# jondo2010/rust-ida

Hardware: AMD Instinct MI355X
Metric: Newton iters/sec (fp64), batched dense DAE N=512 B=4096 (higher is better)
Workload: dtype f64

## Files before the change

### rust-ida_amd/csrc/exp_switches.hpp

```cpp
#pragma once

#if !defined(IDAHIP_TIMING_BUILD) &&                                                                                   \
    (defined(IDAHIP_EXP_NOPRO) || defined(IDAHIP_EXP_NOUPD) || defined(IDAHIP_EXP_NOGATHER) || defined(IDAHIP_EXP_NODIAG) || \
     defined(IDAHIP_EXP_NOSWEEP) || defined(IDAHIP_STAMPS) || defined(IDAHIP_TRAIL_PIPE) || defined(IDAHIP_TRAIL_QUAD) ||   \
     defined(IDAHIP_WP_RING) || defined(IDAHIP_US_PAD) || defined(IDAHIP_SYS_UNR) || defined(IDAHIP_TRAIL_AHEAD) ||         \
     defined(IDAHIP_NT_SYS) || defined(IDAHIP_NT_SOLVE) || defined(IDAHIP_NT_FINALIZE) || defined(IDAHIP_NT_TRAIL))
#error "IDAHIP_EXP_* / IDAHIP_STAMPS / IDAHIP_TRAIL_* (IDAHIP_TRAIL_AHEAD: 0..3) / IDAHIP_WP_RING / IDAHIP_US_PAD / IDAHIP_SYS_UNR / IDAHIP_NT_* are timing-build switches: add -DIDAHIP_TIMING_BUILD (the library then reports itself as one and is not a product)"
#endif

namespace idahip {
namespace tb {

#ifdef IDAHIP_TIMING_BUILD
constexpr bool TIMING_BUILD = true;
#else
constexpr bool TIMING_BUILD = false;
#endif

#ifdef IDAHIP_EXP_NOPRO
constexpr bool NOPRO = true;
#else
constexpr bool NOPRO = false;
#endif
#ifdef IDAHIP_EXP_NOUPD
constexpr bool NOUPD = true;
#else
constexpr bool NOUPD = false;
#endif
#ifdef IDAHIP_EXP_NOGATHER
constexpr bool NOGATHER = true;
#else
constexpr bool NOGATHER = false;
#endif
#ifdef IDAHIP_EXP_NODIAG
constexpr bool NODIAG = true;
#else
constexpr bool NODIAG = false;
#endif
#ifdef IDAHIP_EXP_NOSWEEP
constexpr bool NOSWEEP = true;
#else
constexpr bool NOSWEEP = false;
#endif
#ifdef IDAHIP_STAMPS
constexpr int STAMPS = IDAHIP_STAMPS;
#else
constexpr int STAMPS = -1;
#endif
#ifdef IDAHIP_TRAIL_PIPE
constexpr bool TRAIL_PIPE = IDAHIP_TRAIL_PIPE != 0;
#else
constexpr bool TRAIL_PIPE = true;
#endif
#ifdef IDAHIP_TRAIL_QUAD
constexpr bool TRAIL_QUAD = IDAHIP_TRAIL_QUAD != 0;
#else
constexpr bool TRAIL_QUAD = true;
#endif
#ifdef IDAHIP_US_PAD
constexpr int US_PAD = IDAHIP_US_PAD;
#else
constexpr int US_PAD = 2;
#endif
#ifdef IDAHIP_TRAIL_AHEAD
constexpr int trail_ahead(int kk) { return IDAHIP_TRAIL_AHEAD; }
#else
constexpr int trail_ahead(int kk) { return kk < 32 ? 1 : 3; }
#endif
#ifdef IDAHIP_WP_RING
constexpr bool WP_DEEP_RING = IDAHIP_WP_RING != 0;
#else
constexpr bool WP_DEEP_RING = false;
#endif
#ifdef IDAHIP_SYS_UNR
constexpr int SYS_UNR = IDAHIP_SYS_UNR;
#else
constexpr int SYS_UNR = 16;
#endif

#ifdef IDAHIP_NT_SYS
constexpr bool NT_SYS = IDAHIP_NT_SYS != 0;
#else
constexpr bool NT_SYS = true;
#endif
#ifdef IDAHIP_NT_SOLVE
constexpr bool NT_SOLVE = IDAHIP_NT_SOLVE != 0;
#else
constexpr bool NT_SOLVE = true;
#endif
#ifdef IDAHIP_NT_FINALIZE
constexpr bool NT_FINALIZE = IDAHIP_NT_FINALIZE != 0;
#else
constexpr bool NT_FINALIZE = true;
#endif
#ifdef IDAHIP_NT_TRAIL
constexpr bool NT_TRAIL = IDAHIP_NT_TRAIL != 0;
#else
constexpr bool NT_TRAIL = false;
#endif

}
}
```

### rust-ida_amd/csrc/lu_wavepanel.hpp

```cpp
#pragma once
#include <type_traits>

#include "lu_kernels.hpp"

namespace idahip {

constexpr int WP_MAX_ROWS = 512;
constexpr int WP_RING(int ns) { return !tb::WP_DEEP_RING ? 2 : (ns >= 1 && ns <= 2) ? 8 : (ns >= 3 && ns <= 7) ? 4 : 2; }

template <bool SLOWK, int NS, class... J>
__global__ __launch_bounds__(64, SLOWK ? 1 : (NS > 0 && NS <= 3 ? 4 : 2)) void lu_wavepanel_kernel(LuWs w, const int k0, const J... jarg) {
    constexpr bool JAC = sizeof...(J) == 1;
    constexpr int BIG = 1 << 20;
    if (!SLOWK && w.cnt && (int)blockIdx.x >= *w.cnt) return;
    const int nredo = SLOWK ? w.redo[(k0 >> 6) - LU_REDO_SLOTS] : 0;
  for (int it = blockIdx.x; !SLOWK || it < nredo; it += gridDim.x) {
    const int item = SLOWK ? w.redo[2 * it + 1] : (int)blockIdx.x;
    const int b = w.idx[item];
    if (w.info[b] != 0) {
        if constexpr (SLOWK) continue;
        else return;
    }
    const int n = w.n;
    double* __restrict__ A = w.mats + (long)b * w.mstride;
    int* __restrict__ pos = w.pos + (long)b * n;
    int* __restrict__ live = w.live + (long)b * n;
    int* __restrict__ prow = w.prow + (long)b * n;
    long long* __restrict__ piv = w.piv + (long)b * w.pstride;
    double* __restrict__ l11 = w.l11 + (long)b * L11_STRIDE;

    const __amdgpu_buffer_rsrc_t rsrc = __builtin_amdgcn_make_buffer_rsrc(A, 0, n * n * 8, 0x00020000);
    const int m = n - k0;
    const int wsp = m < 64 ? m : 64;
    const int lane = threadIdx.x;
    const int nslots = NS > 0 ? NS : (m + 63) >> 6;
    constexpr int NSC = NS > 0 ? NS : 8;

    __shared__ int ptab[64];

    int rowid[8], rpos[8], pstep[8];
    unsigned roff[8];
    static_for<0, NSC>([&](auto st) {
        constexpr int S = decltype(st)::value;
        const int li = S * 64 + lane;
        const bool has = li < m;
        rowid[S] = has ? live[li] : 0;
        rpos[S] = has ? pos[rowid[S]] : 0x7fffffff;
        pstep[S] = has ? BIG : -1;
        roff[S] = (unsigned)rowid[S] * 8u;
    });

    const LuJac jq = lu_jac_arg(jarg...);
    double jcj = 0.0;
    __amdgpu_buffer_rsrc_t rsJa = rsrc, rsJb = rsrc;
    if constexpr (JAC) {
        jcj = jq.cj[jq.cj_by_sys ? b : item];
        rsJa = __builtin_amdgcn_make_buffer_rsrc(const_cast<double*>(jq.a) + (long)b * n * n, 0, n * n * 8, 0x00020000);
        rsJb = __builtin_amdgcn_make_buffer_rsrc(const_cast<double*>(jq.b) + (long)b * n * n, 0, n * n * 8, 0x00020000);
    }
    auto load_block_jac = [&](double (&x)[8][8], const int b8, const int wb) {
        constexpr int JT = 2;
        const int coloff = (k0 + b8) * n * 8;
        auto jo = [&](const int j) { return coloff + (j < wb ? j : wb - 1) * n * 8; };
        static_for<0, NSC>([&](auto st) {
            constexpr int S = decltype(st)::value;
#pragma unroll
            for (int j = 0; j < 8; ++j) x[S][j] = buf_load_f64(rsJa, roff[S], jo(j));
        });
        double t[JT][8];
        static_for<0, (JT < NSC ? JT : NSC)>([&](auto st) {
            constexpr int S = decltype(st)::value;
#pragma unroll
            for (int j = 0; j < 8; ++j) t[S][j] = buf_load_f64(rsJb, roff[S], jo(j));
        });
        static_for<0, NSC>([&](auto st) {
            constexpr int S = decltype(st)::value;
#pragma unroll
            for (int j = 0; j < 8; ++j) {
                const double v = t[S % JT][j] + jcj * x[S][j];
                x[S][j] = (S < nslots && j < wb) ? v : 0.0;
            }
            if constexpr (S + JT < NSC) {
                __builtin_amdgcn_sched_barrier(0);
#pragma unroll
                for (int j = 0; j < 8; ++j) t[S % JT][j] = buf_load_f64(rsJb, roff[S + JT], jo(j));
            }
        });
    };
    auto load_block = [&](double (&x)[8][8], const int b8, const int wb) {
        if constexpr (JAC) {
            load_block_jac(x, b8, wb);
        } else {
            static_for<0, NSC>([&](auto st) {
                constexpr int S = decltype(st)::value;
                if (S < nslots) {
                    const double* __restrict__ src = A + (long)(k0 + b8) * n + rowid[S];
#pragma unroll
                    for (int j = 0; j < 8; ++j) x[S][j] = (j < wb) ? src[(long)j * n] : 0.0;
                } else {
#pragma unroll
                    for (int j = 0; j < 8; ++j) x[S][j] = 0.0;
                }
            });
        }
    };
    auto store_block = [&](const double (&x)[8][8], const int b8, const int wb) {
        static_for<0, NSC>([&](auto st) {
            constexpr int S = decltype(st)::value;
            if (S < nslots && pstep[S] >= 0) {
                double* __restrict__ dst = A + (long)(k0 + b8) * n + rowid[S];
#pragma unroll
                for (int j = 0; j < 8; ++j)
                    if (j < wb) dst[(long)j * n] = x[S][j];
            }
        });
    };

    auto process = [&](auto slow_tag, double (&x)[8][8], const int b8, const int wb) -> int {
        constexpr bool SLOW = decltype(slow_tag)::value;
        if (b8 > 0) {
            auto load_l = [&](double (&l)[8], const int k) {
                const int coloff = (k0 + k) * n * 8;
                static_for<0, NSC>([&](auto st) {
                    constexpr int S = decltype(st)::value;
                    l[S] = buf_load_f64(rsrc, roff[S], coloff);
                });
            };
            auto apply = [&](const double (&l)[8], const int k, const int ow) {
                const int pl = __builtin_amdgcn_readfirstlane(ow) & 63, ps = __builtin_amdgcn_readfirstlane(ow) >> 6;
                double uk[8];
                switch (ps) {
#define IDAHIP_WP_CASE(SV)                                                                     \
    case SV:                                                                                   \
        if constexpr (SV < NSC) {                                                              \
            _Pragma("unroll") for (int j = 0; j < 8; ++j) uk[j] = readlane_f64(x[SV][j], pl); \
        }                                                                                      \
        break;
                    IDAHIP_WP_CASE(1)
                    IDAHIP_WP_CASE(2)
                    IDAHIP_WP_CASE(3)
                    IDAHIP_WP_CASE(4)
                    IDAHIP_WP_CASE(5)
                    IDAHIP_WP_CASE(6)
                    IDAHIP_WP_CASE(7)
                    default:
                        IDAHIP_WP_CASE(0)
#undef IDAHIP_WP_CASE
                }
                double ukv[8];
                if (SLOW) {
#pragma unroll
                    for (int j = 0; j < 8; ++j) ukv[j] = opaque_vgpr(uk[j]);
                }
                static_for<0, NSC>([&](auto st) {
                    constexpr int S = decltype(st)::value;
                    if (S < nslots) {
                        if (pstep[S] > k) {
#pragma unroll
                            for (int j = 0; j < 8; ++j) {
                                if (SLOW) {
                                    const double tn = upd(x[S][j], ukv[j], l[S]);
                                    x[S][j] = (ukv[j] == 0.0) ? x[S][j] : tn;
                                } else {
                                    x[S][j] = upd(x[S][j], uk[j], l[S]);
                                }
                            }
                        }
                    }
                });
            };
            __builtin_amdgcn_s_waitcnt(0x0F70);
            constexpr int D = WP_RING(NS);
            double l[D][8];
            int ow[D];
            static_for<0, D>([&](auto dt) {
                constexpr int d = decltype(dt)::value;
                load_l(l[d], d);
                ow[d] = ptab[d];
            });
#pragma unroll 1
            for (int k = 0; k < b8; k += D) {
                static_for<0, D>([&](auto dt) {
                    constexpr int d = decltype(dt)::value;
                    apply(l[d], k + d, ow[d]);
                    const int kn = (k + d + D < b8) ? k + d + D : b8 - 1;
                    load_l(l[d], kn);
                    ow[d] = ptab[kn];
                });
            }
        }
        bool special = false;
        int status = 0, failcol = 0;
        static_for<0, 8>([&](auto kt) {
            constexpr int kk = decltype(kt)::value;
            const bool active = !SLOW || (status == 0 && kk < wb);
            const int kstep = b8 + kk, kc = k0 + kstep;
            unsigned kh[8], kl[8];
            static_for<0, NSC>([&](auto st) {
                constexpr int S = decltype(st)::value;
                const double v = x[S][kk];
                unsigned h = (unsigned)__double2hiint(v) | 0x80000000u, l = (unsigned)__double2loint(v);
                if (SLOW) {
                    if (v != v) {
                        h = (rpos[S] == kc) ? 0xfff00000u : 0u;
                        l = 0u;
                    }
                }
                kh[S] = (pstep[S] == BIG) ? h : 0u;
                kl[S] = l;
            });
            unsigned lm = kh[0];
#pragma unroll
            for (int s = 1; s < NSC; ++s) lm = kh[s] > lm ? kh[s] : lm;
            const unsigned mh = wave_max_u32<false>(lm);
            if (!SLOW) special = special || mh >= 0xfff00000u;
            int cnt = 0, slot = 0;
#pragma unroll
            for (int s = 0; s < NSC; ++s) {
                const bool e = kh[s] == mh;
                cnt += e ? 1 : 0;
                slot = e ? s : slot;
            }
            const unsigned long long bal = __ballot(cnt > 0);
            int pl = (int)__ffsll((unsigned long long)bal) - 1;
            int ps;
            if (__popcll(bal) == 1 && __builtin_amdgcn_readlane(cnt, pl) == 1) {
                ps = __builtin_amdgcn_readlane(slot, pl);
            } else {
                unsigned bl = 0u;
                int bp_ = 0x7fffffff, bs = 0;
#pragma unroll
                for (int s = 0; s < NSC; ++s) {
                    const bool e = kh[s] == mh;
                    const bool better = e && (kl[s] > bl || (kl[s] == bl && rpos[s] < bp_) || bp_ == 0x7fffffff);
                    bl = better ? kl[s] : bl;
                    bp_ = better ? rpos[s] : bp_;
                    bs = better ? s : bs;
                }
                const bool e1 = bp_ != 0x7fffffff;
                const unsigned ml = wave_max_u32<false>(e1 ? bl : 0u);
                const bool top = e1 && bl == ml;
                const int pm = wave_min_i32f<false>(top ? bp_ : 0x7fffffff);
                const unsigned long long b2 = __ballot(top && bp_ == pm);
                pl = (int)__ffsll((unsigned long long)b2) - 1;
                ps = __builtin_amdgcn_readlane(bs, pl);
            }
            double u[8];
            int bp = 0, pr = 0;
            switch (ps) {
#define IDAHIP_WP_CASE(SV)                                                                             \
    case SV:                                                                                           \
        if constexpr (SV < NSC) {                                                                      \
            _Pragma("unroll") for (int j = kk; j < 8; ++j) u[j] = readlane_f64(x[SV][j], pl);         \
            bp = __builtin_amdgcn_readlane(rpos[SV], pl);                                              \
            pr = __builtin_amdgcn_readlane(rowid[SV], pl);                                             \
        }                                                                                              \
        break;
                IDAHIP_WP_CASE(1)
                IDAHIP_WP_CASE(2)
                IDAHIP_WP_CASE(3)
                IDAHIP_WP_CASE(4)
                IDAHIP_WP_CASE(5)
                IDAHIP_WP_CASE(6)
                IDAHIP_WP_CASE(7)
                default:
                    IDAHIP_WP_CASE(0)
#undef IDAHIP_WP_CASE
            }
            bool go = active;
            if (active && u[kk] == 0.0) {
                status = 1;
                failcol = kc + 1;
                go = !SLOW;
            }
            const double recip = 1.0 / u[kk];
            if (go) {
                if (lane == 0) {
                    piv[kc] = (long long)bp;
                    prow[kc] = pr;
                    ptab[kstep] = pl | (ps << 6);
                }
                __builtin_amdgcn_fence(__ATOMIC_RELEASE, "wavefront");
                __builtin_amdgcn_wave_barrier();
                static_for<0, NSC>([&](auto st) {
                    constexpr int S = decltype(st)::value;
                    if (pstep[S] == BIG && rpos[S] == kc) rpos[S] = bp;
                    if (lane == pl && ps == S) {
                        pstep[S] = kstep;
                        rpos[S] = kc;
                    }
                });
            }
            double uv[8];
            if (SLOW) {
#pragma unroll
                for (int j = kk + 1; j < 8; ++j) uv[j] = opaque_vgpr(u[j]);
            }
            static_for<0, NSC>([&](auto st) {
                constexpr int S = decltype(st)::value;
                if (S < nslots) {
                    if (pstep[S] == BIG && go) {
                        const double l = x[S][kk] * recip;
                        x[S][kk] = l;
#pragma unroll
                        for (int j = kk + 1; j < 8; ++j) {
                            if (SLOW) {
                                const double tn = upd(x[S][j], uv[j], l);
                                x[S][j] = (uv[j] == 0.0) ? x[S][j] : tn;
                            } else {
                                x[S][j] = upd(x[S][j], u[j], l);
                            }
                        }
                    }
                }
            });
        });
        if (!SLOW) {
            bool z = false;
            static_for<0, NSC>([&](auto st) {
                constexpr int S = decltype(st)::value;
                bool zz = false;
#pragma unroll
                for (int j = 0; j < 8; ++j) zz = zz || (x[S][j] == 0.0 && j < wb);
                z = z || (zz && pstep[S] >= 0 && pstep[S] != BIG);
            });
            if (special || status != 0 || __ballot(z) != 0ull) return 2;
        }
        if (status == 1 && lane == 0) w.info[b] = failcol;
        return status;
    };

    int bstart = 0;
    if (SLOWK) {
        const int rd = w.redo[2 * b];
        if (rd == 0) continue;
        bstart = (rd - 1) * 8;
        for (int k = 0; k < bstart; ++k) {
            const int kc = k0 + k;
            const int bp = (int)piv[kc], pr = prow[kc];
            static_for<0, NSC>([&](auto st) {
                constexpr int S = decltype(st)::value;
                if (pstep[S] == BIG && rpos[S] == kc) rpos[S] = bp;
                const bool mine = pstep[S] >= 0 && rowid[S] == pr;
                if (mine) {
                    pstep[S] = k;
                    rpos[S] = kc;
                }
                const unsigned long long bm = __ballot(mine);
                if (bm != 0ull && lane == 0) ptab[k] = ((int)__ffsll((unsigned long long)bm) - 1) | (S << 6);
            });
            __builtin_amdgcn_fence(__ATOMIC_RELEASE, "wavefront");
            __builtin_amdgcn_wave_barrier();
        }
        if (lane == 0) w.redo[2 * b] = 0;
    }
    bool zero_pivot = false;
    for (int b8 = bstart; b8 < wsp; b8 += 8) {
        const int wb = (wsp - b8) < 8 ? (wsp - b8) : 8;
        double x[8][8];
        int st;
        if (SLOWK) {
            load_block(x, b8, wb);
            st = process(std::true_type{}, x, b8, wb);
        } else {
            if (wb != 8) {
                st = 2;
            } else {
                load_block(x, b8, 8);
                st = process(std::false_type{}, x, b8, 8);
            }
            if (st == 2) {
                if (lane == 0) {
                    w.redo[2 * b] = 1 + (b8 >> 3);
                    w.redo[2 * atomicAdd(&w.redo[(k0 >> 6) - LU_REDO_SLOTS], 1) + 1] = item;
                }
                return;
            }
        }
        if (st != 0) {
            if constexpr (SLOWK) {
                zero_pivot = true;
                break;
            } else {
                return;
            }
        }
        store_block(x, b8, wb);
    }
    if (SLOWK && zero_pivot) continue;

    __syncthreads();
    static_for<0, NSC>([&](auto st) {
        constexpr int S = decltype(st)::value;
        if (pstep[S] >= 0) pos[rowid[S]] = rpos[S];
    });
    unsigned short* __restrict__ om = w.ord ? w.ord + ((long)b * w.ordq + (k0 >> 6)) * n : nullptr;
    if (lane < wsp) {
        const double* __restrict__ src = A + (long)k0 * n + prow[k0 + lane];
        if (om) {
            double* __restrict__ O = w.out + (long)b * w.ostride + (long)k0 * n + k0 + lane;
            for (int j0 = 0; j0 < wsp; j0 += 8) {
                double v[8];
#pragma unroll
                for (int u = 0; u < 8; ++u) v[u] = (j0 + u < wsp) ? src[(long)(j0 + u) * n] : 0.0;
#pragma unroll
                for (int u = 0; u < 8; ++u)
                    if (j0 + u < wsp) {
                        O[(long)(j0 + u) * n] = v[u];
                        if (j0 + u < lane) l11[(j0 + u) * 64 + lane] = v[u];
                    }
            }
            if (w.perm) w.perm[(long)b * n + k0 + lane] = prow[k0 + lane];
        } else {
            for (int j0 = 0; j0 < lane; j0 += 8) {
                double v[8];
#pragma unroll
                for (int u = 0; u < 8; ++u) v[u] = (j0 + u < lane) ? src[(long)(j0 + u) * n] : 0.0;
#pragma unroll
                for (int u = 0; u < 8; ++u)
                    if (j0 + u < lane) l11[(j0 + u) * 64 + lane] = v[u];
            }
        }
    }
    int base = 0;
    static_for<0, NSC>([&](auto st) {
        constexpr int S = decltype(st)::value;
        const bool al = pstep[S] == BIG;
        const unsigned long long bal = __ballot(al);
        const int rank = base + __popcll(bal & ((1ull << lane) - 1ull));
        if (al) live[rank] = rowid[S];
        if (om && pstep[S] >= 0) om[S * 64 + lane] = (unsigned short)(al ? 64 + rank : pstep[S]);
        base += __popcll(bal);
    });
    if constexpr (!SLOWK) return;
  }
}

}
```

Before: 397,200.

## Widen wave-panel LU column blocks for low-slot fast path

Adds a WP_WIDE switch, enabled by default for one-slot panels, that processes 64, 32 or 16 columns per register block instead of 8 on the fast non-Jacobian path. The kernel adds extra column groups to the pivot update loop and uses buffer loads and stores for the wider blocks. With a 64-wide block it skips the separate left-looking apply phase. The aim is fewer block iterations and less reloading of earlier L columns. The cost is much higher register use (minimum occupancy drops to 2 waves per EU for widened variants) and a partial-tail handoff to the slow kernel.

```diff
diff --git a/rust-ida_amd/csrc/exp_switches.hpp b/rust-ida_amd/csrc/exp_switches.hpp
--- a/rust-ida_amd/csrc/exp_switches.hpp
+++ b/rust-ida_amd/csrc/exp_switches.hpp
@@ -4,8 +4,9 @@
     (defined(IDAHIP_EXP_NOPRO) || defined(IDAHIP_EXP_NOUPD) || defined(IDAHIP_EXP_NOGATHER) || defined(IDAHIP_EXP_NODIAG) || \
      defined(IDAHIP_EXP_NOSWEEP) || defined(IDAHIP_STAMPS) || defined(IDAHIP_TRAIL_PIPE) || defined(IDAHIP_TRAIL_QUAD) ||   \
      defined(IDAHIP_WP_RING) || defined(IDAHIP_US_PAD) || defined(IDAHIP_SYS_UNR) || defined(IDAHIP_TRAIL_AHEAD) ||         \
-     defined(IDAHIP_NT_SYS) || defined(IDAHIP_NT_SOLVE) || defined(IDAHIP_NT_FINALIZE) || defined(IDAHIP_NT_TRAIL))
-#error "IDAHIP_EXP_* / IDAHIP_STAMPS / IDAHIP_TRAIL_* (IDAHIP_TRAIL_AHEAD: 0..3) / IDAHIP_WP_RING / IDAHIP_US_PAD / IDAHIP_SYS_UNR / IDAHIP_NT_* are timing-build switches: add -DIDAHIP_TIMING_BUILD (the library then reports itself as one and is not a product)"
+     defined(IDAHIP_NT_SYS) || defined(IDAHIP_NT_SOLVE) || defined(IDAHIP_NT_FINALIZE) || defined(IDAHIP_NT_TRAIL) ||       \
+     defined(IDAHIP_WP_WIDE))
+#error "IDAHIP_EXP_* / IDAHIP_STAMPS / IDAHIP_TRAIL_* (IDAHIP_TRAIL_AHEAD: 0..3) / IDAHIP_WP_RING / IDAHIP_WP_WIDE / IDAHIP_US_PAD / IDAHIP_SYS_UNR / IDAHIP_NT_* are timing-build switches: add -DIDAHIP_TIMING_BUILD (the library then reports itself as one and is not a product)"
 #endif
 
 namespace idahip {
@@ -72,6 +73,11 @@
 #else
 constexpr bool WP_DEEP_RING = false;
 #endif
+#ifdef IDAHIP_WP_WIDE
+constexpr int WP_WIDE = IDAHIP_WP_WIDE;
+#else
+constexpr int WP_WIDE = 0x01;
+#endif
 #ifdef IDAHIP_SYS_UNR
 constexpr int SYS_UNR = IDAHIP_SYS_UNR;
 #else
diff --git a/rust-ida_amd/csrc/lu_wavepanel.hpp b/rust-ida_amd/csrc/lu_wavepanel.hpp
--- a/rust-ida_amd/csrc/lu_wavepanel.hpp
+++ b/rust-ida_amd/csrc/lu_wavepanel.hpp
@@ -7,10 +7,17 @@
 
 constexpr int WP_MAX_ROWS = 512;
 constexpr int WP_RING(int ns) { return !tb::WP_DEEP_RING ? 2 : (ns >= 1 && ns <= 2) ? 8 : (ns >= 3 && ns <= 7) ? 4 : 2; }
+constexpr int WP_WIDTH(bool slowk, int ns, bool jac) {
+    if (slowk || jac || ns < 1 || ns > 5 || !((tb::WP_WIDE >> (ns - 1)) & 1)) return 8;
+    return ns == 1 ? 64 : ns == 2 ? 32 : 16;
+}
 
 template <bool SLOWK, int NS, class... J>
-__global__ __launch_bounds__(64, SLOWK ? 1 : (NS > 0 && NS <= 3 ? 4 : 2)) void lu_wavepanel_kernel(LuWs w, const int k0, const J... jarg) {
+__global__ __launch_bounds__(64, SLOWK ? 1 : (NS > 0 && NS <= 3 && WP_WIDTH(SLOWK, NS, sizeof...(J) == 1) == 8 ? 4 : 2)) void lu_wavepanel_kernel(LuWs w, const int k0, const J... jarg) {
     constexpr bool JAC = sizeof...(J) == 1;
+    constexpr int W = WP_WIDTH(SLOWK, NS, JAC);
+    constexpr bool RTW = W > 8 && NS == 1;
+    static_assert(W == 8 || (!SLOWK && !JAC && NS >= 1 && NS <= 5 && 64 % W == 0), "wide blocks: FAST, 1..5 slots, J formed");
     constexpr int BIG = 1 << 20;
     if (!SLOWK && w.cnt && (int)blockIdx.x >= *w.cnt) return;
     const int nredo = SLOWK ? w.redo[(k0 >> 6) - LU_REDO_SLOTS] : 0;
@@ -58,7 +65,7 @@
         rsJa = __builtin_amdgcn_make_buffer_rsrc(const_cast<double*>(jq.a) + (long)b * n * n, 0, n * n * 8, 0x00020000);
         rsJb = __builtin_amdgcn_make_buffer_rsrc(const_cast<double*>(jq.b) + (long)b * n * n, 0, n * n * 8, 0x00020000);
     }
-    auto load_block_jac = [&](double (&x)[8][8], const int b8, const int wb) {
+    auto load_block_jac = [&](double (&x)[8][W], const int b8, const int wb) {
         constexpr int JT = 2;
         const int coloff = (k0 + b8) * n * 8;
         auto jo = [&](const int j) { return coloff + (j < wb ? j : wb - 1) * n * 8; };
@@ -87,38 +94,53 @@
             }
         });
     };
-    auto load_block = [&](double (&x)[8][8], const int b8, const int wb) {
+    auto load_block = [&](double (&x)[8][W], const int b8, const int wb) {
         if constexpr (JAC) {
             load_block_jac(x, b8, wb);
+        } else if constexpr (W > 8) {
+            static_for<0, NSC>([&](auto st) {
+                constexpr int S = decltype(st)::value;
+#pragma unroll
+                for (int j = 0; j < W; ++j) {
+                    const double v = buf_load_f64(rsrc, roff[S], (k0 + b8 + (j < wb ? j : wb - 1)) * n * 8);
+                    x[S][j] = (j < wb) ? v : 0.0;
+                }
+            });
         } else {
             static_for<0, NSC>([&](auto st) {
                 constexpr int S = decltype(st)::value;
                 if (S < nslots) {
                     const double* __restrict__ src = A + (long)(k0 + b8) * n + rowid[S];
 #pragma unroll
-                    for (int j = 0; j < 8; ++j) x[S][j] = (j < wb) ? src[(long)j * n] : 0.0;
+                    for (int j = 0; j < W; ++j) x[S][j] = (j < wb) ? src[(long)j * n] : 0.0;
                 } else {
 #pragma unroll
-                    for (int j = 0; j < 8; ++j) x[S][j] = 0.0;
+                    for (int j = 0; j < W; ++j) x[S][j] = 0.0;
                 }
             });
         }
     };
-    auto store_block = [&](const double (&x)[8][8], const int b8, const int wb) {
+    auto store_block = [&](const double (&x)[8][W], const int b8, const int wb) {
         static_for<0, NSC>([&](auto st) {
             constexpr int S = decltype(st)::value;
             if (S < nslots && pstep[S] >= 0) {
-                double* __restrict__ dst = A + (long)(k0 + b8) * n + rowid[S];
-#pragma unroll
-                for (int j = 0; j < 8; ++j)
-                    if (j < wb) dst[(long)j * n] = x[S][j];
+                if constexpr (W > 8) {
+#pragma unroll
+                    for (int j = 0; j < W; ++j)
+                        if (j < wb) buf_store_f64(rsrc, roff[S], (k0 + b8 + j) * n * 8, x[S][j]);
+                } else {
+                    double* __restrict__ dst = A + (long)(k0 + b8) * n + rowid[S];
+#pragma unroll
+                    for (int j = 0; j < 8; ++j)
+                        if (j < wb) dst[(long)j * n] = x[S][j];
+                }
             }
         });
     };
 
-    auto process = [&](auto slow_tag, double (&x)[8][8], const int b8, const int wb) -> int {
+    auto process = [&](auto slow_tag, double (&x)[8][W], const int b8, const int wb) -> int {
         constexpr bool SLOW = decltype(slow_tag)::value;
-        if (b8 > 0) {
+        if (W < 64 && b8 > 0) {
             auto load_l = [&](double (&l)[8], const int k) {
                 const int coloff = (k0 + k) * n * 8;
                 static_for<0, NSC>([&](auto st) {
@@ -128,13 +150,15 @@
             };
             auto apply = [&](const double (&l)[8], const int k, const int ow) {
                 const int pl = __builtin_amdgcn_readfirstlane(ow) & 63, ps = __builtin_amdgcn_readfirstlane(ow) >> 6;
+              static_for<0, W / 8>([&](auto gt) {
+                constexpr int G = decltype(gt)::value * 8;
                 double uk[8];
                 switch (ps) {
-#define IDAHIP_WP_CASE(SV)                                                                     \
-    case SV:                                                                                   \
-        if constexpr (SV < NSC) {                                                              \
-            _Pragma("unroll") for (int j = 0; j < 8; ++j) uk[j] = readlane_f64(x[SV][j], pl); \
-        }                                                                                      \
+#define IDAHIP_WP_CASE(SV)                                                                         \
+    case SV:                                                                                       \
+        if constexpr (SV < NSC) {                                                                  \
+            _Pragma("unroll") for (int j = 0; j < 8; ++j) uk[j] = readlane_f64(x[SV][G + j], pl); \
+        }                                                                                          \
         break;
                     IDAHIP_WP_CASE(1)
                     IDAHIP_WP_CASE(2)
@@ -159,15 +183,16 @@
 #pragma unroll
                             for (int j = 0; j < 8; ++j) {
                                 if (SLOW) {
-                                    const double tn = upd(x[S][j], ukv[j], l[S]);
-                                    x[S][j] = (ukv[j] == 0.0) ? x[S][j] : tn;
+                                    const double tn = upd(x[S][G + j], ukv[j], l[S]);
+                                    x[S][G + j] = (ukv[j] == 0.0) ? x[S][G + j] : tn;
                                 } else {
-                                    x[S][j] = upd(x[S][j], uk[j], l[S]);
+                                    x[S][G + j] = upd(x[S][G + j], uk[j], l[S]);
                                 }
                             }
                         }
                     }
                 });
+              });
             };
             __builtin_amdgcn_s_waitcnt(0x0F70);
             constexpr int D = WP_RING(NS);
@@ -191,8 +216,12 @@
         }
         bool special = false;
         int status = 0, failcol = 0;
-        static_for<0, 8>([&](auto kt) {
+        static_for<0, W>([&](auto kt) {
             constexpr int kk = decltype(kt)::value;
+            constexpr int GE = (kk | 7) + 1;
+            if constexpr (RTW) {
+                if ((kk & ~7) >= wb) return;
+            }
             const bool active = !SLOW || (status == 0 && kk < wb);
             const int kstep = b8 + kk, kc = k0 + kstep;
             unsigned kh[8], kl[8];
@@ -251,7 +280,7 @@
 #define IDAHIP_WP_CASE(SV)                                                                             \
     case SV:                                                                                           \
         if constexpr (SV < NSC) {                                                                      \
-            _Pragma("unroll") for (int j = kk; j < 8; ++j) u[j] = readlane_f64(x[SV][j], pl);         \
+            _Pragma("unroll") for (int j = kk; j < GE; ++j) u[j & 7] = readlane_f64(x[SV][j], pl);    \
             bp = __builtin_amdgcn_readlane(rpos[SV], pl);                                              \
             pr = __builtin_amdgcn_readlane(rowid[SV], pl);                                             \
         }                                                                                              \
@@ -268,12 +297,12 @@
 #undef IDAHIP_WP_CASE
             }
             bool go = active;
-            if (active && u[kk] == 0.0) {
+            if (active && u[kk & 7] == 0.0) {
                 status = 1;
                 failcol = kc + 1;
                 go = !SLOW;
             }
-            const double recip = 1.0 / u[kk];
+            const double recip = 1.0 / u[kk & 7];
             if (go) {
                 if (lane == 0) {
                     piv[kc] = (long long)bp;
@@ -294,7 +323,7 @@
             double uv[8];
             if (SLOW) {
 #pragma unroll
-                for (int j = kk + 1; j < 8; ++j) uv[j] = opaque_vgpr(u[j]);
+                for (int j = kk + 1; j < GE; ++j) uv[j & 7] = opaque_vgpr(u[j & 7]);
             }
             static_for<0, NSC>([&](auto st) {
                 constexpr int S = decltype(st)::value;
@@ -303,16 +332,47 @@
                         const double l = x[S][kk] * recip;
                         x[S][kk] = l;
 #pragma unroll
-                        for (int j = kk + 1; j < 8; ++j) {
+                        for (int j = kk + 1; j < GE; ++j) {
                             if (SLOW) {
-                                const double tn = upd(x[S][j], uv[j], l);
-                                x[S][j] = (uv[j] == 0.0) ? x[S][j] : tn;
+                                const double tn = upd(x[S][j], uv[j & 7], l);
+                                x[S][j] = (uv[j & 7] == 0.0) ? x[S][j] : tn;
                             } else {
-                                x[S][j] = upd(x[S][j], u[j], l);
+                                x[S][j] = upd(x[S][j], u[j & 7], l);
                             }
                         }
                     }
                 }
+            });
+            static_for<GE / 8, W / 8>([&](auto gt) {
+                constexpr int G = decltype(gt)::value * 8;
+                if constexpr (RTW) {
+                    if (G >= wb) return;
+                }
+                double ug[8];
+                switch (ps) {
+#define IDAHIP_WP_CASE(SV)                                                                         \
+    case SV:                                                                                       \
+        if constexpr (SV < NSC) {                                                                  \
+            _Pragma("unroll") for (int j = 0; j < 8; ++j) ug[j] = readlane_f64(x[SV][G + j], pl); \
+        }                                                                                          \
+        break;
+                    IDAHIP_WP_CASE(1)
+                    IDAHIP_WP_CASE(2)
+                    IDAHIP_WP_CASE(3)
+                    IDAHIP_WP_CASE(4)
+                    default:
+                        IDAHIP_WP_CASE(0)
+#undef IDAHIP_WP_CASE
+                }
+                static_for<0, NSC>([&](auto st) {
+                    constexpr int S = decltype(st)::value;
+                    if (S < nslots) {
+                        if (pstep[S] == BIG && go) {
+#pragma unroll
+                            for (int j = 0; j < 8; ++j) x[S][G + j] = upd(x[S][G + j], ug[j], x[S][kk]);
+                        }
+                    }
+                });
             });
         });
         if (!SLOW) {
@@ -320,8 +380,14 @@
             static_for<0, NSC>([&](auto st) {
                 constexpr int S = decltype(st)::value;
                 bool zz = false;
-#pragma unroll
-                for (int j = 0; j < 8; ++j) zz = zz || (x[S][j] == 0.0 && j < wb);
+                if constexpr (W == 8) {
+#pragma unroll
+                    for (int j = 0; j < 8; ++j) zz = zz || (x[S][j] == 0.0 && j < wb);
+                } else {
+                    const int pc = pstep[S] - b8;
+#pragma unroll
+                    for (int j = 0; j < W; ++j) zz = zz || (x[S][j] == 0.0 && j < wb && j > pc);
+                }
                 z = z || (zz && pstep[S] >= 0 && pstep[S] != BIG);
             });
             if (special || status != 0 || __ballot(z) != 0ull) return 2;
@@ -355,23 +421,39 @@
         if (lane == 0) w.redo[2 * b] = 0;
     }
     bool zero_pivot = false;
-    for (int b8 = bstart; b8 < wsp; b8 += 8) {
-        const int wb = (wsp - b8) < 8 ? (wsp - b8) : 8;
-        double x[8][8];
+    for (int b8 = bstart; b8 < wsp; b8 += W) {
+        const int wb = (wsp - b8) < W ? (wsp - b8) : W;
+        double x[8][W];
         int st;
+        int hand = b8;
         if (SLOWK) {
             load_block(x, b8, wb);
             st = process(std::true_type{}, x, b8, wb);
         } else {
-            if (wb != 8) {
-                st = 2;
+            if constexpr (W == 8) {
+                if (wb != 8) {
+                    st = 2;
+                } else {
+                    load_block(x, b8, 8);
+                    st = process(std::false_type{}, x, b8, 8);
+                }
             } else {
-                load_block(x, b8, 8);
-                st = process(std::false_type{}, x, b8, 8);
+                const int wf = RTW ? (wb & ~7) : W;
+                if (wf == 0) {
+                    st = 2;
+                } else {
+                    load_block(x, b8, wf);
+                    st = process(std::false_type{}, x, b8, wf);
+                    if (RTW && st == 0 && wf != wb) {
+                        store_block(x, b8, wf);
+                        hand = b8 + wf;
+                        st = 2;
+                    }
+                }
             }
             if (st == 2) {
                 if (lane == 0) {
-                    w.redo[2 * b] = 1 + (b8 >> 3);
+                    w.redo[2 * b] = 1 + (hand >> 3);
                     w.redo[2 * atomicAdd(&w.redo[(k0 >> 6) - LU_REDO_SLOTS], 1) + 1] = item;
                 }
                 return;
```

Result: no change. 397,100 (-0.0%).
